# nju-ee/MODE-2022

Hardware: AMD Instinct MI355X
Metric: ERP stereo pairs/sec (512x1024, 192 disp) fwd+bwd (higher is better)
Workload: dtype fp32 storage/accumulate; products: 2xfp16 split (22-bit, per-tensor 2^k scale, 3 MFMAs) in the stride-1 3x3x3 / spherical / 3x3 layers incl. gradients (DESIGN 3u/3v); 3xbf16 split (24-bit, 6 MFMAs) in the stride-2 / transposed 3x3x3 layers and the polar spherical tiles (3j-3l); fp32 MFMA in the 32->; 1 GPU; ModeDisparity(192,Sphere,1024x512 Cassini) fwd+bwd+Adam step, batch 2/GPU (BASELINE configs[2]); global_batch=2, conv_arith=bf16x6, init=recipe state, seed 1 (tests/golden/recipe.py), parallelism=dp1

## Files before the change

mode-2022_amd/csrc/sphere_conv.hip:

```cpp
#include <cstring>

#include "common.h"
#include "sphere_internal.h"

namespace {

typedef float f32x16 __attribute__((ext_vector_type(16)));

constexpr int P = 64;
constexpr int CCH = 8;
constexpr int NTHREADS = 256;

struct Dims {
  int B, Ci, H, W, Co, KK, sH, sW, Ho, Wo, G;
  int Cig, Cog;
  int npix;
  int tps;
  int MT;
  int NCHUNK;
  int CB;
  int NB;
  int KSQ;
  int accumulate;
};
// ... 304 lines not shown
      for (int e = 0; e < s.y; ++e) {
        const int2 ent = entries[s.x + e];
        const float wt = __int_as_float(ent.y);
        v0 += wt * g0[ent.x];
        v1 += wt * g1[ent.x];
      }
      buf[((qd * 2) * d.KK + k) * P + p] = ok0 ? v0 : 0.f;
      buf[((qd * 2 + 1) * d.KK + k) * P + p] = ok1 ? v1 : 0.f;
    }
  };

  f32x16 acc0 = {0}, acc1 = {0};
  const float4* wpa = wp + ((long long)(g * MTc + (active ? mt : 0)) * NCHo) * d.KK * 64 + lane;

  produce(0, colbuf);
  __syncthreads();
  for (int ch = 0; ch < NCHo; ++ch) {
    float* cur = colbuf + (ch & 1) * rows * P;
    if (ch + 1 < NCHo) produce(ch + 1, colbuf + ((ch + 1) & 1) * rows * P);
    if (active) {
      const float4* wq = wpa + (long long)ch * d.KK * 64;
      const float* bp = cur + (lane >> 5) * P + (lane & 31);
      for (int quad = 0; quad < d.KK; ++quad) {
        const float4 a4 = wq[quad * 64];
        const float* bq = bp + quad * 8 * P;
        acc0 = mfma32(a4.x, bq[0], acc0);
        acc1 = mfma32(a4.x, bq[32], acc1);
        acc0 = mfma32(a4.y, bq[2 * P], acc0);
        acc1 = mfma32(a4.y, bq[2 * P + 32], acc1);
        acc0 = mfma32(a4.z, bq[4 * P], acc0);
        acc1 = mfma32(a4.z, bq[4 * P + 32], acc1);
        acc0 = mfma32(a4.w, bq[6 * P], acc0);
        acc1 = mfma32(a4.w, bq[6 * P + 32], acc1);
      }
    }
    __syncthreads();
  }

  if (active) {
    float* gxb = gx + ((long long)b * d.Ci + (long long)g * d.Cig) * HWin;
#pragma unroll
    for (int r = 0; r < 16; ++r) {
      const int c = mt * 32 + (r & 3) + 8 * (r >> 2) + 4 * (lane >> 5);
      if (c < d.Cig) {
        const int qq = q0 + (lane & 31);
        float* o0 = gxb + (long long)c * HWin + qq;
        if (qq < HWin) o0[0] = d.accumulate ? o0[0] + acc0[r] : acc0[r];
        if (qq + 32 < HWin) o0[32] = d.accumulate ? o0[32] + acc1[r] : acc1[r];
      }
    }
  }
}

__global__ __launch_bounds__(NTHREADS) void sphere_bwd_data_adj9_kernel(const float* __restrict__ gy, const int* __restrict__ rowptr,
                                                                         const int2* __restrict__ entries,
                                                                         const float4* __restrict__ wp, float* __restrict__ gx, Dims d,
                                                                         int MTc, int NCHo, int qtiles, const int* __restrict__ tile_list) {
  constexpr int KT = 9, EC = 4;
  extern __shared__ __attribute__((aligned(16))) char smem[];
  int4* ent_p = reinterpret_cast<int4*>(smem);
  float4* ent_w = reinterpret_cast<float4*>(smem + KT * P * 16);
  int2* span = reinterpret_cast<int2*>(smem + KT * P * 32);
  float* colbuf = reinterpret_cast<float*>(smem + KT * P * 40);
  constexpr int rows = CCH * KT;
  const int HWin = d.H * d.W;

  const int tile = xcd_remap(blockIdx.x, gridDim.x);
  const int b = tile / qtiles;
  const int q0 = (tile_list ? tile_list[tile - b * qtiles] : tile - b * qtiles) * P;
  const int g = blockIdx.z;
  const int tid = threadIdx.x;
  const int wave = tid >> 6, lane = tid & 63;
  const int mt = blockIdx.y * 4 + wave;
  const bool active = mt < MTc;

  for (int item = tid; item < KT * P; item += NTHREADS) {
    const int k = item / P, pp = item % P;
    const int qq = q0 + pp;
    int beg = 0, cnt = 0;
    if (qq < HWin) {
      beg = rowptr[(long long)k * HWin + qq];
      cnt = rowptr[(long long)k * HWin + qq + 1] - beg;
    }
    int pe[EC];
    float we[EC];
#pragma unroll
    for (int e = 0; e < EC; ++e) {
      const int2 ent = entries[beg + min(e, max(cnt - 1, 0))];
      pe[e] = e < cnt ? ent.x * 4 : 0;
      we[e] = e < cnt ? __int_as_float(ent.y) : 0.f;
    }
    ent_p[item] = make_int4(pe[0], pe[1], pe[2], pe[3]);
    ent_w[item] = make_float4(we[0], we[1], we[2], we[3]);
    span[item] = make_int2(beg, cnt);
  }
  __syncthreads();

  const int p = tid & (P - 1);
  static_assert(P == 64, "one wave per output-channel pair of the chunk");
  const int qd = __builtin_amdgcn_readfirstlane(tid / P);
  const float* gyg = gy + ((long long)b * d.Co + (long long)g * d.Cog) * d.npix;
  float lv[KT * 2 * EC];
  bool has_tail = false;
#pragma unroll
  for (int k = 0; k < KT; ++k) has_tail |= span[k * P + p].y > EC;

  auto issue = [&](int ch) {
    const int o0 = ch * CCH + qd * 2;
    const float* g0 = gyg + (long long)(o0 < d.Cog ? o0 : 0) * d.npix;
    const float* g1 = gyg + (long long)(o0 + 1 < d.Cog ? o0 + 1 : 0) * d.npix;
#pragma unroll
    for (int k = 0; k < KT; ++k) {
      const int4 pe = ent_p[k * P + p];
      const char* c0 = reinterpret_cast<const char*>(g0);
      const char* c1 = reinterpret_cast<const char*>(g1);
#define MODE_LD(base, off) (*reinterpret_cast<const float*>((base) + (unsigned)(off)))
      lv[k * 8 + 0] = MODE_LD(c0, pe.x); lv[k * 8 + 1] = MODE_LD(c0, pe.y); lv[k * 8 + 2] = MODE_LD(c0, pe.z); lv[k * 8 + 3] = MODE_LD(c0, pe.w);
      lv[k * 8 + 4] = MODE_LD(c1, pe.x); lv[k * 8 + 5] = MODE_LD(c1, pe.y); lv[k * 8 + 6] = MODE_LD(c1, pe.z); lv[k * 8 + 7] = MODE_LD(c1, pe.w);
#undef MODE_LD
    }
  };
  auto finish = [&](int ch, float* buf) {
    const int o0 = ch * CCH + qd * 2;
    const bool ok0 = o0 < d.Cog, ok1 = o0 + 1 < d.Cog;
    const float* g0 = gyg + (long long)(ok0 ? o0 : 0) * d.npix;
    const float* g1 = gyg + (long long)(ok1 ? o0 + 1 : 0) * d.npix;
    float v0[KT], v1[KT];
#pragma unroll
    for (int k = 0; k < KT; ++k) {
      const float4 we = ent_w[k * P + p];
      float a = we.x * lv[k * 8 + 0];
      float b = we.x * lv[k * 8 + 4];
      asm volatile("" : "+v"(a), "+v"(b));
      a = fmaf(we.y, lv[k * 8 + 1], a);
      b = fmaf(we.y, lv[k * 8 + 5], b);
      asm volatile("" : "+v"(a), "+v"(b));
      a = fmaf(we.z, lv[k * 8 + 2], a);
      b = fmaf(we.z, lv[k * 8 + 6], b);
      asm volatile("" : "+v"(a), "+v"(b));
      a = fmaf(we.w, lv[k * 8 + 3], a);
      b = fmaf(we.w, lv[k * 8 + 7], b);
      asm volatile("" : "+v"(a), "+v"(b));
      v0[k] = a;
      v1[k] = b;
    }
    if (has_tail) {
#pragma unroll
      for (int k = 0; k < KT; ++k) {
        const int2 s = span[k * P + p];
        for (int e = EC; e < s.y; ++e) {
          const int2 ent = entries[s.x + e];
          const float wt = __int_as_float(ent.y);
          float a = g0[ent.x], b = g1[ent.x];
          asm volatile("" : "+v"(a), "+v"(b));
          v0[k] = fmaf(wt, a, v0[k]);
          asm volatile("" : "+v"(v0[k]));
          v1[k] = fmaf(wt, b, v1[k]);
        }
      }
    }
#pragma unroll
    for (int k = 0; k < KT; ++k) {
      buf[((qd * 2) * KT + k) * P + p] = ok0 ? v0[k] : 0.f;
      buf[((qd * 2 + 1) * KT + k) * P + p] = ok1 ? v1[k] : 0.f;
    }
  };

  f32x16 acc0 = {0}, acc1 = {0};
  const float4* wpa = wp + ((long long)(g * MTc + (active ? mt : 0)) * NCHo) * KT * 64 + lane;

  float4 wcur[KT], wnxt[KT];
#pragma unroll
  for (int quad = 0; quad < KT; ++quad) wcur[quad] = wpa[quad * 64];
  issue(0);
  finish(0, colbuf);
  __syncthreads();
  for (int ch = 0; ch < NCHo; ++ch) {
    float* cur = colbuf + (ch & 1) * rows * P;
    float* nxt = colbuf + ((ch + 1) & 1) * rows * P;
    if (ch + 1 < NCHo) {
      const float4* wq = wpa + (long long)(ch + 1) * KT * 64;
#pragma unroll
      for (int quad = 0; quad < KT; ++quad) wnxt[quad] = wq[quad * 64];
      issue(ch + 1);
    }
    if (active) {
      const float* bp = cur + (lane >> 5) * P + (lane & 31);
      float bn[8];
#pragma unroll
      for (int i = 0; i < 8; ++i) bn[i] = bp[(i >> 1) * 2 * P + (i & 1) * 32];
#pragma unroll
      for (int quad = 0; quad < KT; ++quad) {
        const float4 a4 = wcur[quad];
        float bc[8];
#pragma unroll
        for (int i = 0; i < 8; ++i) bc[i] = bn[i];
        if (quad + 1 < KT) {
          const float* bq = bp + (quad + 1) * 8 * P;
#pragma unroll
          for (int i = 0; i < 8; ++i) bn[i] = bq[(i >> 1) * 2 * P + (i & 1) * 32];
        }
        __builtin_amdgcn_sched_barrier(0);
        acc0 = mfma32(a4.x, bc[0], acc0);
        acc1 = mfma32(a4.x, bc[1], acc1);
        acc0 = mfma32(a4.y, bc[2], acc0);
        acc1 = mfma32(a4.y, bc[3], acc1);
        acc0 = mfma32(a4.z, bc[4], acc0);
        acc1 = mfma32(a4.z, bc[5], acc1);
        acc0 = mfma32(a4.w, bc[6], acc0);
        acc1 = mfma32(a4.w, bc[7], acc1);
      }
    }
    if (ch + 1 < NCHo) {
      finish(ch + 1, nxt);
#pragma unroll
      for (int quad = 0; quad < KT; ++quad) wcur[quad] = wnxt[quad];
    }
    __syncthreads();
  }

  if (active) {
    float* gxb = gx + ((long long)b * d.Ci + (long long)g * d.Cig) * HWin;
#pragma unroll
    for (int r = 0; r < 16; ++r) {
      const int c = mt * 32 + (r & 3) + 8 * (r >> 2) + 4 * (lane >> 5);
      if (c < d.Cig) {
        const int qq = q0 + (lane & 31);
        float* o0 = gxb + (long long)c * HWin + qq;
        if (qq < HWin) o0[0] = d.accumulate ? o0[0] + acc0[r] : acc0[r];
        if (qq + 32 < HWin) o0[32] = d.accumulate ? o0[32] + acc1[r] : acc1[r];
      }
    }
  }
}

__global__ __launch_bounds__(NTHREADS) void sphere_bwd_data_kernel(const float* __restrict__ gy, const float* __restrict__ pos,
                                                                    const float4* __restrict__ wp, float* __restrict__ gx,
                                                                    Dims d) {
  extern __shared__ __attribute__((aligned(16))) char smem[];
  float4* tap_w = reinterpret_cast<float4*>(smem);
  unsigned* tap_off = reinterpret_cast<unsigned*>(smem + (size_t)d.KK * P * 16);
  float* gyl = reinterpret_cast<float*>(smem + (size_t)d.KK * P * 20);

  const int tile = xcd_remap(blockIdx.x, gridDim.x);
  const int b = tile / d.tps;
  const int pix0 = (tile - b * d.tps) * P;
  const int g = blockIdx.z;
  const int tid = threadIdx.x;
  const int wave = tid >> 6, lane = tid & 63;

  compute_tapinfo(pos, d, pix0, tap_off, tap_w);
  const float* gyb = gy + ((long long)b * d.Co + (long long)g * d.Cog) * d.npix;
  for (int idx = tid; idx < d.KSQ * 8 * P; idx += NTHREADS) {
    const int co = idx / P, p = idx % P;
    float v = 0.f;
    if (co < d.Cog && pix0 + p < d.npix) v = gyb[(long long)co * d.npix + pix0 + p];
    gyl[idx] = v;
  }
  __syncthreads();

  const long long HW = (long long)d.H * d.W;
  float* gxg = gx + ((long long)b * d.Ci + (long long)g * d.Cig) * HW;
  const float* bp = gyl + (lane >> 5) * P + (lane & 31);
  const int nrows = d.CB * d.KK;

  for (int nb = 0; nb < d.NB; ++nb) {
    f32x16 acc0 = {0}, acc1 = {0};
    const float4* wq = wp + ((long long)((g * d.NB + nb) * 4 + wave) * d.KSQ) * 64 + lane;
    for (int ks4 = 0; ks4 < d.KSQ; ++ks4) {
      const float4 a4 = wq[ks4 * 64];
      const float* bq = bp + ks4 * 8 * P;
      acc0 = mfma32(a4.x, bq[0], acc0);
      acc1 = mfma32(a4.x, bq[32], acc1);
      acc0 = mfma32(a4.y, bq[2 * P], acc0);
      acc1 = mfma32(a4.y, bq[2 * P + 32], acc1);
      acc0 = mfma32(a4.z, bq[4 * P], acc0);
      acc1 = mfma32(a4.z, bq[4 * P + 32], acc1);
      acc0 = mfma32(a4.w, bq[6 * P], acc0);
      acc1 = mfma32(a4.w, bq[6 * P + 32], acc1);
    }
#pragma unroll
    for (int r = 0; r < 16; ++r) {
      const int rr = wave * 32 + (r & 3) + 8 * (r >> 2) + 4 * (lane >> 5);
// ... 361 lines not shown
    for (int p = 0; p < npix; ++p) {
      const int n = corners(k, p, qs, ws);
      for (int i = 0; i < n; ++i) {
        const int32_t at = rowptr_host[(long long)k * HW + qs[i]]++;
        entries_host[2 * (long long)at] = p;
        int32_t bits;
        memcpy(&bits, &ws[i], 4);
        entries_host[2 * (long long)at + 1] = bits;
      }
    }
  for (long long i = nrows; i > 0; --i) rowptr_host[i] = rowptr_host[i - 1];
  rowptr_host[0] = 0;
  return MODE_OK;
}

static int bwd_data_adj_impl(const float* gy, const float* w, float* gx, float* wpack, const int32_t* adj_rowptr,
                             const int32_t* adj_entries, int B, int Ci, int H, int W, int Co, int Kh, int Kw, int Ho, int Wo, int groups,
                             int accumulate, const int32_t* tile_list, int n_list, mode_stream_t stream);

extern "C" int mode_sphere_conv_bwd_data_adj(const float* gy, const float* w, float* gx, float* wpack, const int32_t* adj_rowptr,
                                             const int32_t* adj_entries, int B, int Ci, int H, int W, int Co, int Kh, int Kw,
                                             int Ho, int Wo, int groups, int accumulate, mode_stream_t stream) {
  return bwd_data_adj_impl(gy, w, gx, wpack, adj_rowptr, adj_entries, B, Ci, H, W, Co, Kh, Kw, Ho, Wo, groups, accumulate, nullptr, 0, stream);
}

extern "C" int mode_sphere_conv_bwd_data_adj_list(const float* gy, const float* w, float* gx, float* wpack, const int32_t* adj_rowptr,
                                                  const int32_t* adj_entries, int B, int Ci, int H, int W, int Co, int Kh, int Kw,
                                                  int Ho, int Wo, int groups, int accumulate, const int32_t* tile_list, int n_list,
                                                  mode_stream_t stream) {
  MODE_REQUIRE(Kh * Kw == 9, MODE_ERR_UNSUPPORTED, "mode_sphere_conv_bwd_data_adj_list: 3x3 kernels only");
  MODE_REQUIRE(n_list >= 0 && (n_list == 0 || tile_list), MODE_ERR_BAD_ARG, "mode_sphere_conv_bwd_data_adj_list: bad tile list");
  if (n_list == 0) return MODE_OK;
  return bwd_data_adj_impl(gy, w, gx, wpack, adj_rowptr, adj_entries, B, Ci, H, W, Co, Kh, Kw, Ho, Wo, groups, accumulate, tile_list, n_list,
                           stream);
}

static int bwd_data_adj_impl(const float* gy, const float* w, float* gx, float* wpack, const int32_t* adj_rowptr,
                             const int32_t* adj_entries, int B, int Ci, int H, int W, int Co, int Kh, int Kw, int Ho, int Wo, int groups,
                             int accumulate, const int32_t* tile_list, int n_list, mode_stream_t stream) {
  Dims d;
  int rc = make_dims(d, B, Ci, H, W, Co, Kh, Kw, 1, 1, Ho, Wo, groups, "mode_sphere_conv_bwd_data_adj");
  if (rc != MODE_OK) return rc;
  d.accumulate = accumulate ? 1 : 0;
  if (B == 0) return MODE_OK;
  MODE_REQUIRE(gy && w && gx && wpack && adj_rowptr && adj_entries, MODE_ERR_BAD_ARG, "mode_sphere_conv_bwd_data_adj: null pointer");
  hipStream_t st = mode::as_stream(stream);
  const int MTc = mode::cdiv(d.Cig, 32);
  const int NCHo = mode::cdiv(d.Cog, CCH);
  const long long npack = (long long)d.G * MTc * NCHo * d.KK * 256;
  if (mode::pack_needed()) hipLaunchKernelGGL(pack_w_adj, dim3(mode::cdiv(npack, 256)), dim3(256), 0, st, w, wpack, d, MTc, NCHo);
  const int qtiles = tile_list ? n_list : mode::cdiv((long long)H * W, P);
  const dim3 grid(B * qtiles, mode::cdiv(MTc, 4), d.G);
  if (d.KK == 9) {
    const size_t lds = (size_t)9 * P * 40 + 2 * (size_t)CCH * 9 * P * 4;
    rc = mode::allow_lds(sphere_bwd_data_adj9_kernel, lds, "mode_sphere_conv_bwd_data_adj");
    if (rc != MODE_OK) return rc;
    hipLaunchKernelGGL(sphere_bwd_data_adj9_kernel, grid, dim3(NTHREADS), lds, st, gy, adj_rowptr,
                       reinterpret_cast<const int2*>(adj_entries), reinterpret_cast<const float4*>(wpack), gx, d, MTc, NCHo, qtiles, tile_list);
  } else {
    const size_t lds = (size_t)d.KK * P * 8 + 2 * (size_t)CCH * d.KK * P * 4;
    rc = mode::allow_lds(sphere_bwd_data_adj_kernel, lds, "mode_sphere_conv_bwd_data_adj");
    if (rc != MODE_OK) return rc;
    hipLaunchKernelGGL(sphere_bwd_data_adj_kernel, grid, dim3(NTHREADS), lds, st, gy, adj_rowptr,
                       reinterpret_cast<const int2*>(adj_entries), reinterpret_cast<const float4*>(wpack), gx, d, MTc, NCHo, qtiles);
  }
  return mode::check_launch("mode_sphere_conv_bwd_data_adj");
}
```

mode-2022_amd/csrc/sphere_conv_win.hip:

```cpp
#include <algorithm>
#include <cstring>
#include <vector>

#include "common.h"
#include "bn_internal.h"
#include "sphere_internal.h"
#include "sphere_tap.h"

namespace {

typedef float f32x16 __attribute__((ext_vector_type(16)));
typedef float f32x32 __attribute__((ext_vector_type(32)));

constexpr int RB = 2;
constexpr int TH = 32 * RB;
constexpr int TW = 4;
constexpr int WC = 8;
constexpr int CCH = 8;
constexpr int KT = 9;
constexpr int MTW = 4;
constexpr int NTHREADS = 64 * TW * RB;
constexpr int SROWS = NTHREADS / WC;
constexpr int WR_SMALL = TH + 17, WR_MID = TH + 81;
constexpr int WR_PIPE_MAX = 5 * SROWS;
// ... 1882 lines not shown
        const uint4* ga = reinterpret_cast<const uint4*>(gyb + (m8 * 32 + j) * BS_GP + 8 * ks8 + 4 * half);
        const uint4 a1 = ga[0], a2 = ga[128 * BS_GP / 4];
        if constexpr (F16) {
          acc8 = sp_mfma_f16(a2, b8[0], acc8);
          acc8 = sp_mfma_f16(a1, b8[1], acc8);
          acc8 = sp_mfma_f16(a1, b8[0], acc8);
        } else {
          const uint4 a3 = ga[2 * (128 * BS_GP / 4)];
          acc8 = sp_mfma(a3, b8[0], acc8);
          acc8 = sp_mfma(a1, b8[2], acc8);
          acc8 = sp_mfma(a2, b8[1], acc8);
          acc8 = sp_mfma(a2, b8[0], acc8);
          acc8 = sp_mfma(a1, b8[1], acc8);
          acc8 = sp_mfma(a1, b8[0], acc8);
        }
      }
      if (more_items) commit_xw(smem + (xbuf ^ 1) * BW_XW, wc);

      __syncthreads();
      if (have_next) commit_col(gpf[(wc + 1) & 1]);
      __syncthreads();
      if (have_next) sample(last_col ? smem + (xbuf ^ 1) * BW_XW : xw, prw0, pro0, b0);
    }
    cur = nxt;
    xbuf ^= 1;
  }
#undef MODE_BS_SPREAD

  float* pb = part + ((((long long)s * gridDim.z + blockIdx.z) * NCG + cg) * BW_SLOTS) * (128 * BW_CG);
#pragma unroll
  for (int m = 0; m < 4; ++m)
#pragma unroll
    for (int r = 0; r < 16; ++r) {
      const int o = m * 32 + (r & 3) + 8 * (r >> 2) + 4 * half;
      pb[((long long)wave * 128 + o) * BW_CG + j] = F16 ? acc[m][r] * unscale : acc[m][r];
    }
  float* red = smem;
  if (wave < 4) {
#pragma unroll
    for (int r = 0; r < 16; ++r) red[(m8 * 32 + (r & 3) + 8 * (r >> 2) + 4 * half) * BW_CG + j] = F16 ? acc8[r] * unscale : acc8[r];
  }
  __syncthreads();
  if (wave >= 4) {
#pragma unroll
    for (int r = 0; r < 16; ++r) red[(m8 * 32 + (r & 3) + 8 * (r >> 2) + 4 * half) * BW_CG + j] += F16 ? acc8[r] * unscale : acc8[r];
  }
  __syncthreads();
  for (int i = tid; i < 128 * BW_CG; i += NTHREADS) pb[(long long)8 * 128 * BW_CG + i] = red[i];
}

constexpr int BQ_X = ((BP_XW + 3) / 4) * 4;
constexpr int BQ_LDS_DWORDS = BQ_X + BS_GYB + 8 * BS_SCR;

__global__ __launch_bounds__(NTHREADS) void sphere_bww_polar_split_kernel(const float* __restrict__ gy, const float* __restrict__ x,
                                                                           float* __restrict__ part, WinDims d,
                                                                           const int* __restrict__ pitems, const float4* __restrict__ rec_w,
                                                                           const int* __restrict__ rec_off, int nitems, int S, int s_base) {
  extern __shared__ __attribute__((aligned(16))) float smem[];
  float* xw = smem;
  uint32_t* gyb = reinterpret_cast<uint32_t*>(smem + BQ_X);
  constexpr int WRP = BP_WR, CP = BP_CP;
  const int s = blockIdx.x, cg = blockIdx.y;
  const int g = blockIdx.z / d.MG, mg = blockIdx.z % d.MG;
  const int tid = threadIdx.x;
  const int wave = tid >> 6, lane = tid & 63;
  const int j = lane & 31, half = lane >> 5;
  float* scr = smem + BQ_X + BS_GYB + wave * BS_SCR;
  const long long HW = (long long)d.H * d.W;
  const int T = nitems * d.B;
  const int omax = d.Cog - mg * 128, cmax = d.Cig - cg * BW_CG;
  const int sh = half, sq = j >> 3, sp8 = j & 7;
  const int ks8 = wave >> 2, m8 = wave & 3;
  const int gpp = tid & 15, go0 = tid >> 4;

  f32x16 acc[4], acc8;
#pragma unroll
  for (int r = 0; r < 16; ++r) {
    acc[0][r] = acc[1][r] = acc[2][r] = acc[3][r] = 0.f;
    acc8[r] = 0.f;
  }
  for (int i = tid; i < BQ_LDS_DWORDS; i += NTHREADS) smem[i] = 0.f;

  constexpr int NE = KT * BP_TAPW;
  const int e0 = tid, e1 = tid + NTHREADS;
  const bool has1 = e1 < NE;
  const int k0 = e0 / BP_TAPW, k1 = (has1 ? e1 : 0) / BP_TAPW;
  const int col0 = (e0 % BP_TAPW) / BP_WR, r0 = e0 % BP_WR;
  const int col1 = ((has1 ? e1 : 0) % BP_TAPW) / BP_WR, r1 = (has1 ? e1 : 0) % BP_WR;

  auto sample = [&](const float4 w4, const int ro, uint4 (&bf)[3]) {
    const float* xb = xw + (8 * sq) * CP + ro;
    float v[8];
#pragma unroll
    for (int c = 0; c < 8; ++c) {
      const float* q = xb + c * CP;
      v[c] = __builtin_fmaf(w4.w, q[WRP + 1], __builtin_fmaf(w4.z, q[1], __builtin_fmaf(w4.y, q[WRP], w4.x * q[0])));
      asm("" : "+v"(v[c]));
    }
    float* sw = scr + (8 * sq) * BS_SCRP + 8 * sh + sp8;
#pragma unroll
    for (int c = 0; c < 8; ++c) sw[c * BS_SCRP] = v[c];
    const float* sr = scr + j * BS_SCRP + 8 * half;
    float t8[8];
#pragma unroll
    for (int i = 0; i < 8; ++i) t8[i] = sr[i];
    uint32_t q1[4], q2[4], q3[4];
#pragma unroll
    for (int i = 0; i < 4; ++i) sp_split2(t8[2 * i], t8[2 * i + 1], q1[i], q2[i], q3[i]);
    bf[0] = make_uint4(q1[0], q1[1], q1[2], q1[3]);
    bf[1] = make_uint4(q2[0], q2[1], q2[2], q2[3]);
    bf[2] = make_uint4(q3[0], q3[1], q3[2], q3[3]);
  };
  auto load_a = [&](int ks, uint4 (&a)[4][3]) {
#pragma unroll
    for (int m = 0; m < 4; ++m) {
      const uint4* ga = reinterpret_cast<const uint4*>(gyb + (m * 32 + j) * BS_GP + 8 * ks + 4 * half);
#pragma unroll
      for (int p = 0; p < 3; ++p) a[m][p] = ga[p * (128 * BS_GP / 4)];
    }
  };
  auto mma24 = [&](const uint4 (&a)[4][3], const uint4 (&bf)[3]) {
#define MODE_BS_TERM(PA, PB) _Pragma("unroll") for (int m = 0; m < 4; ++m) acc[m] = sp_mfma(a[m][PA], bf[PB], acc[m]);
    MODE_BS_TERM(2, 0)
    MODE_BS_TERM(0, 2)
    MODE_BS_TERM(1, 1)
    MODE_BS_TERM(1, 0)
    MODE_BS_TERM(0, 1)
    MODE_BS_TERM(0, 0)
#undef MODE_BS_TERM
  };

  for (int t = s; t < T; t += S) {
    const int b = t / nitems, it = t - b * nitems;
    const int* pi = pitems + (long long)it * BP_ITEM_INTS;
    const int h0 = pi[0], w = pi[1];
    __syncthreads();
    {
      const int rb0 = pi[2 + k0], cb0 = pi[2 + KT + k0], rb1 = pi[2 + k1], cb1 = pi[2 + KT + k1];
      const bool ok0 = cb0 + col0 < d.W, ok1 = has1 && cb1 + col1 < d.W;
      const float* xg = x + ((long long)b * d.Ci + (long long)g * d.Cig + (long long)cg * BW_CG) * HW;
      const long long a0 = ok0 ? (long long)((rb0 + r0) % d.H) * d.sh + (long long)(cb0 + col0) * d.sw : 0;
      const long long a1 = ok1 ? (long long)((rb1 + r1) % d.H) * d.sh + (long long)(cb1 + col1) * d.sw : 0;
#pragma unroll 1
      for (int c8 = 0; c8 < BW_CG; c8 += 8) {
        float v0[8], v1[8];
#pragma unroll
        for (int c = 0; c < 8; ++c) {
          const long long co = (long long)min(c8 + c, cmax - 1) * HW;
          v0[c] = xg[co + a0];
          v1[c] = xg[co + a1];
        }
#pragma unroll
        for (int c = 0; c < 8; ++c) {
          xw[(c8 + c) * BP_CP + e0] = (ok0 && c8 + c < cmax) ? v0[c] : 0.f;
          if (has1) xw[(c8 + c) * BP_CP + e1] = (ok1 && c8 + c < cmax) ? v1[c] : 0.f;
        }
      }
    }
    {
      const int h = h0 + 2 * gpp;
      const bool ok0 = h < d.H && w < d.W, ok1 = h + 1 < d.H && w < d.W;
      const float* gyb0 = gy + ((long long)b * d.Co + (long long)g * d.Cog + (long long)mg * 128) * HW +
                          (ok0 ? (long long)h * d.sh + (long long)w * d.sw : 0);
      const long long step1 = ok1 ? d.sh : 0;
      float v0[4], v1[4];
#pragma unroll
      for (int u = 0; u < 4; ++u) {
        const float* p = gyb0 + (long long)min(go0 + 32 * u, omax - 1) * HW;
        v0[u] = p[0];
        v1[u] = p[step1];
      }
#pragma unroll
      for (int u = 0; u < 4; ++u) {
        const bool oo = go0 + 32 * u < omax;
        uint32_t p1, p2, p3;
        sp_split2((ok0 && oo) ? v0[u] : 0.f, (ok1 && oo) ? v1[u] : 0.f, p1, p2, p3);
        uint32_t* dst = gyb + (go0 + 32 * u) * BS_GP + gpp;
        dst[0] = p1;
        dst[128 * BS_GP] = p2;
        dst[2 * 128 * BS_GP] = p3;
      }
    }
    const long long rbase = (long long)it * BW_NREC;
    const int px0 = 8 * sh + sp8;
    const float4 rw0 = rec_w[rbase + wave * BW_TH + px0], rw1 = rec_w[rbase + wave * BW_TH + 16 + px0];
    const float4 rw8 = rec_w[rbase + 8 * BW_TH + 16 * ks8 + px0];
    const int ro0 = rec_off[rbase + wave * BW_TH + px0], ro1 = rec_off[rbase + wave * BW_TH + 16 + px0];
    const int ro8 = rec_off[rbase + 8 * BW_TH + 16 * ks8 + px0];
    __syncthreads();
    uint4 a[4][3], b0[3], b1[3], b8[3];
    sample(rw0, ro0, b0);
    load_a(0, a);
    sample(rw1, ro1, b1);
    mma24(a, b0);
    load_a(1, a);
    sample(rw8, ro8, b8);
    mma24(a, b1);
    {
      const uint4* ga = reinterpret_cast<const uint4*>(gyb + (m8 * 32 + j) * BS_GP + 8 * ks8 + 4 * half);
      const uint4 a1 = ga[0], a2 = ga[128 * BS_GP / 4], a3 = ga[2 * (128 * BS_GP / 4)];
      acc8 = sp_mfma(a3, b8[0], acc8);
      acc8 = sp_mfma(a1, b8[2], acc8);
      acc8 = sp_mfma(a2, b8[1], acc8);
      acc8 = sp_mfma(a2, b8[0], acc8);
      acc8 = sp_mfma(a1, b8[1], acc8);
      acc8 = sp_mfma(a1, b8[0], acc8);
    }
  }
  __syncthreads();
  float* pb = part + ((((long long)(s_base + s) * gridDim.z + blockIdx.z) * gridDim.y + cg) * BW_SLOTS) * (128 * BW_CG);
#pragma unroll
  for (int m = 0; m < 4; ++m)
#pragma unroll
    for (int r = 0; r < 16; ++r) {
      const int o = m * 32 + (r & 3) + 8 * (r >> 2) + 4 * half;
      pb[((long long)wave * 128 + o) * BW_CG + j] = acc[m][r];
    }
  float* red = smem;
  if (wave < 4) {
#pragma unroll
    for (int r = 0; r < 16; ++r) red[(m8 * 32 + (r & 3) + 8 * (r >> 2) + 4 * half) * BW_CG + j] = acc8[r];
  }
  __syncthreads();
  if (wave >= 4) {
#pragma unroll
    for (int r = 0; r < 16; ++r) red[(m8 * 32 + (r & 3) + 8 * (r >> 2) + 4 * half) * BW_CG + j] += acc8[r];
  }
  __syncthreads();
  for (int i = tid; i < 128 * BW_CG; i += NTHREADS) pb[(long long)8 * 128 * BW_CG + i] = red[i];
}

size_t win_lds_bytes(int wr, bool pipe) { return ((size_t)(pipe ? 2 : 1) * CCH * chan_pitch(wr) + wr + 8) * sizeof(float); }
constexpr size_t TALL_W_BYTES = 2 * (size_t)MTW * 3 * 64 * sizeof(uint4);
size_t tall_split_lds_bytes(int wr) { return ((win_lds_bytes(wr, true) + 15) / 16) * 16 + TALL_W_BYTES; }
bool wrap_is_pipelined(int H) { return H + 1 <= WR_PIPE_MAX && win_lds_bytes(H + 1, true) <= 160 * 1024; }

__global__ __launch_bounds__(256) void transpose_planes_kernel(const float* __restrict__ in, float* __restrict__ out, int H, int W) {
  __shared__ float tile[32][33];
  const long long plane = (long long)blockIdx.z * H * W;
  const int w0 = blockIdx.x * 32, h0 = blockIdx.y * 32;
  const int tx = threadIdx.x & 31, ty = threadIdx.x >> 5;
#pragma unroll
  for (int i = 0; i < 32; i += 8) {
    const int h = h0 + ty + i, w = w0 + tx;
    if (h < H && w < W) tile[ty + i][tx] = in[plane + (long long)h * W + w];
  }
  __syncthreads();
#pragma unroll
  for (int i = 0; i < 32; i += 8) {
    const int w = w0 + ty + i, h = h0 + tx;
    if (h < H && w < W) out[plane + (long long)w * H + h] = tile[tx][ty + i];
  }
}

int make_win_dims(WinDims& d, int B, int Ci, int H, int W, int Co, int Kh, int Kw, int groups, const char* who) {
  MODE_REQUIRE(B >= 0 && Ci > 0 && H > 0 && W > 0 && Co > 0 && groups > 0, MODE_ERR_BAD_ARG, "%s: non-positive size", who);
  MODE_REQUIRE(Kh * Kw == KT, MODE_ERR_UNSUPPORTED, "%s: the windowed kernels are built for %d taps (got %dx%d)", who, KT, Kh, Kw);
  MODE_REQUIRE(Ci % groups == 0 && Co % groups == 0, MODE_ERR_BAD_ARG, "%s: channels not divisible by groups", who);
  MODE_REQUIRE((long long)H * W < (1LL << 30), MODE_ERR_UNSUPPORTED, "%s: image too large", who);
  d.B = B; d.Ci = Ci; d.H = H; d.W = W; d.Co = Co; d.G = groups;
  d.Cig = Ci / groups;
  d.Cog = Co / groups;
  d.NCH = mode::cdiv(d.Cig, CCH);
  d.MG = mode::cdiv(d.Cog, 128);
  d.wr = H + 1;
  d.sh = W;
  d.sw = 1;
  d.wrap_pipe = wrap_is_pipelined(H) ? 1 : 0;
  d.accumulate = 0;
  return MODE_OK;
}


}

extern "C" size_t mode_sphere_plan_max_tiles(int H, int W) {
  if (H <= 0 || W <= 0) return 0;
  return (size_t)mode::cdiv(H, TH) * mode::cdiv(W, TW);
}
// ... 414 lines not shown
  MODE_REQUIRE((amax_g == nullptr) == (amax_x == nullptr), MODE_ERR_BAD_ARG, "mode_sphere_conv_bwd_weight_win: both operand maxima, or neither");
  if (rc != MODE_OK) return rc;
  MODE_REQUIRE((gy_t == nullptr) == (x_t == nullptr), MODE_ERR_BAD_ARG, "mode_sphere_conv_bwd_weight_win: gy_t and x_t come together");
  if (gy_t) {
    d.sh = 1;
    d.sw = H;
  }
  MODE_REQUIRE(n_small >= 0 && n_mid >= 0 && n_wrap >= 0 && n_rest_pixels >= 0 && n_polar_items >= 0 &&
                   (size_t)n_small + n_mid + n_wrap == mode_sphere_plan_max_tiles(H, W),
               MODE_ERR_BAD_ARG, "mode_sphere_conv_bwd_weight_win: the plan must cover every tile");
  if (B == 0) return MODE_OK;
  MODE_REQUIRE(((gy && x) || (gy_t && n_rest_pixels == 0)) && pos && gw && workspace && tiles && (n_rest_pixels == 0 || rest_pixels) &&
                   (n_small == 0 || (rec_w && rec_off)) &&
                   (n_polar_items == 0 || (pitems && prec_w && prec_off)),
               MODE_ERR_BAD_ARG, "mode_sphere_conv_bwd_weight_win: null pointer");
  hipStream_t st = mode::as_stream(stream);
  const int NCG = mode::cdiv(d.Cig, BW_CG);
  const size_t slice = (size_t)d.G * d.MG * NCG * BW_SLOTS * 128 * BW_CG * sizeof(float);
  const float* gys = gy_t ? gy_t : gy;
  const float* xs = x_t ? x_t : x;
  int S = 0;
  if (n_small > 0) {
    S = bww_win_splits(d, n_small);
    if (split) {
      const size_t lds = (size_t)BS_LDS_DWORDS * sizeof(float);
      if (amax_g) {
        rc = mode::allow_lds(sphere_bww_split_kernel<true>, lds, "mode_sphere_conv_bwd_weight_win_split");
        if (rc != MODE_OK) return rc;
        hipLaunchKernelGGL(sphere_bww_split_kernel<true>, dim3(S, NCG, d.G * d.MG), dim3(NTHREADS), lds, st, gys, xs, workspace, d,
                           reinterpret_cast<const int4*>(tiles) + n_wrap + n_mid, reinterpret_cast<const float4*>(rec_w), rec_off, n_small, S,
                           amax_g, amax_x);
      } else {
        rc = mode::allow_lds(sphere_bww_split_kernel<false>, lds, "mode_sphere_conv_bwd_weight_win_split");
        if (rc != MODE_OK) return rc;
        hipLaunchKernelGGL(sphere_bww_split_kernel<false>, dim3(S, NCG, d.G * d.MG), dim3(NTHREADS), lds, st, gys, xs, workspace, d,
                           reinterpret_cast<const int4*>(tiles) + n_wrap + n_mid, reinterpret_cast<const float4*>(rec_w), rec_off, n_small, S,
                           amax_g, amax_x);
      }
    } else {
      const size_t lds = (size_t)BW_LDS_FLOATS * sizeof(float);
      rc = mode::allow_lds(sphere_bww_win_kernel, lds, "mode_sphere_conv_bwd_weight_win");
      if (rc != MODE_OK) return rc;
      hipLaunchKernelGGL(sphere_bww_win_kernel, dim3(S, NCG, d.G * d.MG), dim3(NTHREADS), lds, st, gys, xs, workspace, d,
                         reinterpret_cast<const int4*>(tiles) + n_wrap + n_mid, reinterpret_cast<const float4*>(rec_w), rec_off, n_small, S);
    }
    rc = mode::check_launch("mode_sphere_conv_bwd_weight_win");
    if (rc != MODE_OK) return rc;
  }
  int Sp = 0;
  if (n_polar_items > 0) {
    Sp = bww_polar_splits(d, n_polar_items);
    if (split) {
      const size_t lds = (size_t)BQ_LDS_DWORDS * sizeof(float);
      rc = mode::allow_lds(sphere_bww_polar_split_kernel, lds, "mode_sphere_conv_bwd_weight_win_split");
      if (rc != MODE_OK) return rc;
      hipLaunchKernelGGL(sphere_bww_polar_split_kernel, dim3(Sp, NCG, d.G * d.MG), dim3(NTHREADS), lds, st, gys, xs, workspace, d, pitems,
                         reinterpret_cast<const float4*>(prec_w), prec_off, n_polar_items, Sp, S);
    } else {
      const size_t lds = (size_t)BP_LDS_FLOATS * sizeof(float);
      rc = mode::allow_lds(sphere_bww_polar_kernel, lds, "mode_sphere_conv_bwd_weight_win");
      if (rc != MODE_OK) return rc;
      hipLaunchKernelGGL(sphere_bww_polar_kernel, dim3(Sp, NCG, d.G * d.MG), dim3(NTHREADS), lds, st, gys, xs, workspace, d, pitems,
                         reinterpret_cast<const float4*>(prec_w), prec_off, n_polar_items, Sp, S);
    }
    rc = mode::check_launch("mode_sphere_conv_bwd_weight_win(polar)");
    if (rc != MODE_OK) return rc;
  }
  if (S + Sp > 0) {
    const long long n = (long long)d.G * d.MG * NCG * KT * 128 * BW_CG;
    hipLaunchKernelGGL(reduce_gw_win, dim3(mode::cdiv(n, 256)), dim3(256), 0, st, workspace, gw, d, S + Sp, NCG);
    rc = mode::check_launch("mode_sphere_conv_bwd_weight_win(reduce)");
    if (rc != MODE_OK) return rc;
  }
  if (n_rest_pixels > 0)
    return mode::sphere_bwd_weight_general(gy, pos, x, gw, reinterpret_cast<float*>(reinterpret_cast<char*>(workspace) + slice * (S + Sp)), B,
                                           Ci, H, W, Co, Kh, Kw, 1, 1, H, W, groups, rest_pixels, n_rest_pixels, st,
                                           "mode_sphere_conv_bwd_weight_win(rest)");
  return MODE_OK;
}

extern "C" int mode_transpose_planes(const float* in, float* out, long long planes, int H, int W, mode_stream_t stream) {
  MODE_REQUIRE(planes >= 0 && H > 0 && W > 0, MODE_ERR_BAD_ARG, "mode_transpose_planes: bad size");
  if (planes == 0) return MODE_OK;
  MODE_REQUIRE(in && out, MODE_ERR_BAD_ARG, "mode_transpose_planes: null pointer");
  hipStream_t st = mode::as_stream(stream);
  for (long long p0 = 0; p0 < planes; p0 += 65535) {
    const int np = (int)std::min<long long>(65535, planes - p0);
    hipLaunchKernelGGL(transpose_planes_kernel, dim3(mode::cdiv(W, 32), mode::cdiv(H, 32), np), dim3(256), 0, st,
                       in + p0 * (long long)H * W, out + p0 * (long long)H * W, H, W);
  }
  return mode::check_launch("mode_transpose_planes");
}

namespace {

constexpr int AJ_PIX = TH * TW;

template <int NS, bool F16>
__device__ __forceinline__ void bwd_data_tile(const float* __restrict__ gy, const uint4* __restrict__ wps, float* __restrict__ gx,
                                              const WinDims& d , int NCH16, const int4 t,
                                              const int4* __restrict__ rec_off, const float4* __restrict__ rec_w,
                                              const int2* __restrict__ rec_off2, const float2* __restrict__ rec_w2, float* smem,
                                              float sx, float unscale) {
  constexpr int WRP = WR_SMALL, CP = SP_CP;
  uint4* opbuf = reinterpret_cast<uint4*>(smem + SP_WIN_FLOATS);
  const int h0 = t.x, w0 = t.y, rbase = t.z, cbase = t.w & 0xffff;
  const int b = blockIdx.y;
  const int g = blockIdx.z / d.MG, mg = blockIdx.z % d.MG;
  const int tid = threadIdx.x, wave = tid >> 6, lane = tid & 63, half = lane >> 5;
  const long long HW = (long long)d.H * d.W;
// ... 634 lines not shown
```

Measured before the change: 35.67 pairs/s.

## Halve adj9 backward-data tile to 32 pixels; add opt-in fp16 polar weight-grad kernel

The 9-tap adjacency backward-data kernel now handles 32-pixel half tiles, giving each thread one output channel instead of two and launching twice as many blocks. This shrinks per-thread register and LDS footprint and should raise occupancy, at the cost of duplicated weight loads and per-block setup. Separately, the polar split weight-gradient kernel is templated with an fp16 2-term split path (3 MFMAs instead of 6) that uses per-tensor scales. That path is enabled only through the MODE_SPHERE_POLAR_F16 environment variable.

```diff
diff --git a/mode-2022_amd/csrc/sphere_conv.hip b/mode-2022_amd/csrc/sphere_conv.hip
--- a/mode-2022_amd/csrc/sphere_conv.hip
+++ b/mode-2022_amd/csrc/sphere_conv.hip
@@ -380,30 +380,35 @@
   }
 }
 
+constexpr int PH = 32;
 __global__ __launch_bounds__(NTHREADS) void sphere_bwd_data_adj9_kernel(const float* __restrict__ gy, const int* __restrict__ rowptr,
                                                                          const int2* __restrict__ entries,
                                                                          const float4* __restrict__ wp, float* __restrict__ gx, Dims d,
                                                                          int MTc, int NCHo, int qtiles, const int* __restrict__ tile_list) {
   constexpr int KT = 9, EC = 4;
+  static_assert(NTHREADS == CCH * PH, "one thread per (output channel of the chunk, pixel of the half tile)");
+  static_assert(P == 2 * PH, "two half tiles per listed tile");
   extern __shared__ __attribute__((aligned(16))) char smem[];
   int4* ent_p = reinterpret_cast<int4*>(smem);
-  float4* ent_w = reinterpret_cast<float4*>(smem + KT * P * 16);
-  int2* span = reinterpret_cast<int2*>(smem + KT * P * 32);
-  float* colbuf = reinterpret_cast<float*>(smem + KT * P * 40);
+  float4* ent_w = reinterpret_cast<float4*>(smem + KT * PH * 16);
+  int2* span = reinterpret_cast<int2*>(smem + KT * PH * 32);
+  float* colbuf = reinterpret_cast<float*>(smem + KT * PH * 40);
   constexpr int rows = CCH * KT;
   const int HWin = d.H * d.W;
 
-  const int tile = xcd_remap(blockIdx.x, gridDim.x);
-  const int b = tile / qtiles;
-  const int q0 = (tile_list ? tile_list[tile - b * qtiles] : tile - b * qtiles) * P;
+  const int htile = xcd_remap(blockIdx.x, gridDim.x);
+  const int b = htile / (2 * qtiles);
+  const int hrem = htile - b * 2 * qtiles;
+  const int q0 = (tile_list ? tile_list[hrem >> 1] : hrem >> 1) * P + (hrem & 1) * PH;
+  if (q0 >= HWin) return;
   const int g = blockIdx.z;
   const int tid = threadIdx.x;
   const int wave = tid >> 6, lane = tid & 63;
   const int mt = blockIdx.y * 4 + wave;
   const bool active = mt < MTc;
 
-  for (int item = tid; item < KT * P; item += NTHREADS) {
-    const int k = item / P, pp = item % P;
+  for (int item = tid; item < KT * PH; item += NTHREADS) {
+    const int k = item / PH, pp = item % PH;
     const int qq = q0 + pp;
     int beg = 0, cnt = 0;
     if (qq < HWin) {
@@ -424,77 +429,62 @@
   }
   __syncthreads();
 
-  const int p = tid & (P - 1);
-  static_assert(P == 64, "one wave per output-channel pair of the chunk");
-  const int qd = __builtin_amdgcn_readfirstlane(tid / P);
+  const int p = tid & (PH - 1);
+  const int cc = tid / PH;
   const float* gyg = gy + ((long long)b * d.Co + (long long)g * d.Cog) * d.npix;
-  float lv[KT * 2 * EC];
+  float lv[KT * EC];
   bool has_tail = false;
 #pragma unroll
-  for (int k = 0; k < KT; ++k) has_tail |= span[k * P + p].y > EC;
+  for (int k = 0; k < KT; ++k) has_tail |= span[k * PH + p].y > EC;
 
   auto issue = [&](int ch) {
-    const int o0 = ch * CCH + qd * 2;
-    const float* g0 = gyg + (long long)(o0 < d.Cog ? o0 : 0) * d.npix;
-    const float* g1 = gyg + (long long)(o0 + 1 < d.Cog ? o0 + 1 : 0) * d.npix;
+    const int o0 = ch * CCH + cc;
+    const char* c0 = reinterpret_cast<const char*>(gyg + (long long)(o0 < d.Cog ? o0 : 0) * d.npix);
 #pragma unroll
     for (int k = 0; k < KT; ++k) {
-      const int4 pe = ent_p[k * P + p];
-      const char* c0 = reinterpret_cast<const char*>(g0);
-      const char* c1 = reinterpret_cast<const char*>(g1);
+      const int4 pe = ent_p[k * PH + p];
 #define MODE_LD(base, off) (*reinterpret_cast<const float*>((base) + (unsigned)(off)))
-      lv[k * 8 + 0] = MODE_LD(c0, pe.x); lv[k * 8 + 1] = MODE_LD(c0, pe.y); lv[k * 8 + 2] = MODE_LD(c0, pe.z); lv[k * 8 + 3] = MODE_LD(c0, pe.w);
-      lv[k * 8 + 4] = MODE_LD(c1, pe.x); lv[k * 8 + 5] = MODE_LD(c1, pe.y); lv[k * 8 + 6] = MODE_LD(c1, pe.z); lv[k * 8 + 7] = MODE_LD(c1, pe.w);
+      lv[k * 4 + 0] = MODE_LD(c0, pe.x); lv[k * 4 + 1] = MODE_LD(c0, pe.y); lv[k * 4 + 2] = MODE_LD(c0, pe.z); lv[k * 4 + 3] = MODE_LD(c0, pe.w);
 #undef MODE_LD
     }
   };
   auto finish = [&](int ch, float* buf) {
-    const int o0 = ch * CCH + qd * 2;
-    const bool ok0 = o0 < d.Cog, ok1 = o0 + 1 < d.Cog;
+    const int o0 = ch * CCH + cc;
+    const bool ok0 = o0 < d.Cog;
     const float* g0 = gyg + (long long)(ok0 ? o0 : 0) * d.npix;
-    const float* g1 = gyg + (long long)(ok1 ? o0 + 1 : 0) * d.npix;
-    float v0[KT], v1[KT];
+    float v0[KT];
 #pragma unroll
     for (int k = 0; k < KT; ++k) {
-      const float4 we = ent_w[k * P + p];
-      float a = we.x * lv[k * 8 + 0];
-      float b = we.x * lv[k * 8 + 4];
-      asm volatile("" : "+v"(a), "+v"(b));
-      a = fmaf(we.y, lv[k * 8 + 1], a);
-      b = fmaf(we.y, lv[k * 8 + 5], b);
-      asm volatile("" : "+v"(a), "+v"(b));
-      a = fmaf(we.z, lv[k * 8 + 2], a);
-      b = fmaf(we.z, lv[k * 8 + 6], b);
-      asm volatile("" : "+v"(a), "+v"(b));
-      a = fmaf(we.w, lv[k * 8 + 3], a);
-      b = fmaf(we.w, lv[k * 8 + 7], b);
-      asm volatile("" : "+v"(a), "+v"(b));
+      const float4 we = ent_w[k * PH + p];
+      float a = we.x * lv[k * 4 + 0];
+      asm volatile("" : "+v"(a));
+      a = fmaf(we.y, lv[k * 4 + 1], a);
+      asm volatile("" : "+v"(a));
+      a = fmaf(we.z, lv[k * 4 + 2], a);
+      asm volatile("" : "+v"(a));
+      a = fmaf(we.w, lv[k * 4 + 3], a);
+      asm volatile("" : "+v"(a));
       v0[k] = a;
-      v1[k] = b;
     }
     if (has_tail) {
 #pragma unroll
       for (int k = 0; k < KT; ++k) {
-        const int2 s = span[k * P + p];
+        const int2 s = span[k * PH + p];
         for (int e = EC; e < s.y; ++e) {
           const int2 ent = entries[s.x + e];
           const float wt = __int_as_float(ent.y);
-          float a = g0[ent.x], b = g1[ent.x];
-          asm volatile("" : "+v"(a), "+v"(b));
+          float a = g0[ent.x];
+          asm volatile("" : "+v"(a));
           v0[k] = fmaf(wt, a, v0[k]);
           asm volatile("" : "+v"(v0[k]));
-          v1[k] = fmaf(wt, b, v1[k]);
         }
       }
     }
 #pragma unroll
-    for (int k = 0; k < KT; ++k) {
-      buf[((qd * 2) * KT + k) * P + p] = ok0 ? v0[k] : 0.f;
-      buf[((qd * 2 + 1) * KT + k) * P + p] = ok1 ? v1[k] : 0.f;
-    }
+    for (int k = 0; k < KT; ++k) buf[(cc * KT + k) * PH + p] = ok0 ? v0[k] : 0.f;
   };
 
-  f32x16 acc0 = {0}, acc1 = {0};
+  f32x16 acc0 = {0};
   const float4* wpa = wp + ((long long)(g * MTc + (active ? mt : 0)) * NCHo) * KT * 64 + lane;
 
   float4 wcur[KT], wnxt[KT];
@@ -504,8 +494,8 @@
   finish(0, colbuf);
   __syncthreads();
   for (int ch = 0; ch < NCHo; ++ch) {
-    float* cur = colbuf + (ch & 1) * rows * P;
-    float* nxt = colbuf + ((ch + 1) & 1) * rows * P;
+    float* cur = colbuf + (ch & 1) * rows * PH;
+    float* nxt = colbuf + ((ch + 1) & 1) * rows * PH;
     if (ch + 1 < NCHo) {
       const float4* wq = wpa + (long long)(ch + 1) * KT * 64;
 #pragma unroll
@@ -513,30 +503,26 @@
       issue(ch + 1);
     }
     if (active) {
-      const float* bp = cur + (lane >> 5) * P + (lane & 31);
-      float bn[8];
-#pragma unroll
-      for (int i = 0; i < 8; ++i) bn[i] = bp[(i >> 1) * 2 * P + (i & 1) * 32];
+      const float* bp = cur + (lane >> 5) * PH + (lane & 31);
+      float bn[4];
+#pragma unroll
+      for (int i = 0; i < 4; ++i) bn[i] = bp[i * 2 * PH];
 #pragma unroll
       for (int quad = 0; quad < KT; ++quad) {
         const float4 a4 = wcur[quad];
-        float bc[8];
-#pragma unroll
-        for (int i = 0; i < 8; ++i) bc[i] = bn[i];
+        float bc[4];
+#pragma unroll
+        for (int i = 0; i < 4; ++i) bc[i] = bn[i];
         if (quad + 1 < KT) {
-          const float* bq = bp + (quad + 1) * 8 * P;
-#pragma unroll
-          for (int i = 0; i < 8; ++i) bn[i] = bq[(i >> 1) * 2 * P + (i & 1) * 32];
+          const float* bq = bp + (quad + 1) * 8 * PH;
+#pragma unroll
+          for (int i = 0; i < 4; ++i) bn[i] = bq[i * 2 * PH];
         }
         __builtin_amdgcn_sched_barrier(0);
         acc0 = mfma32(a4.x, bc[0], acc0);
-        acc1 = mfma32(a4.x, bc[1], acc1);
-        acc0 = mfma32(a4.y, bc[2], acc0);
-        acc1 = mfma32(a4.y, bc[3], acc1);
-        acc0 = mfma32(a4.z, bc[4], acc0);
-        acc1 = mfma32(a4.z, bc[5], acc1);
-        acc0 = mfma32(a4.w, bc[6], acc0);
-        acc1 = mfma32(a4.w, bc[7], acc1);
+        acc0 = mfma32(a4.y, bc[1], acc0);
+        acc0 = mfma32(a4.z, bc[2], acc0);
+        acc0 = mfma32(a4.w, bc[3], acc0);
       }
     }
     if (ch + 1 < NCHo) {
@@ -549,14 +535,13 @@
 
   if (active) {
     float* gxb = gx + ((long long)b * d.Ci + (long long)g * d.Cig) * HWin;
+    const int qq = q0 + (lane & 31);
 #pragma unroll
     for (int r = 0; r < 16; ++r) {
       const int c = mt * 32 + (r & 3) + 8 * (r >> 2) + 4 * (lane >> 5);
-      if (c < d.Cig) {
-        const int qq = q0 + (lane & 31);
+      if (c < d.Cig && qq < HWin) {
         float* o0 = gxb + (long long)c * HWin + qq;
-        if (qq < HWin) o0[0] = d.accumulate ? o0[0] + acc0[r] : acc0[r];
-        if (qq + 32 < HWin) o0[32] = d.accumulate ? o0[32] + acc1[r] : acc1[r];
+        o0[0] = d.accumulate ? o0[0] + acc0[r] : acc0[r];
       }
     }
   }
@@ -1024,10 +1009,12 @@
   const int qtiles = tile_list ? n_list : mode::cdiv((long long)H * W, P);
   const dim3 grid(B * qtiles, mode::cdiv(MTc, 4), d.G);
   if (d.KK == 9) {
-    const size_t lds = (size_t)9 * P * 40 + 2 * (size_t)CCH * 9 * P * 4;
+    MODE_REQUIRE((long long)B * qtiles * 2 < (1ll << 31), MODE_ERR_UNSUPPORTED, "mode_sphere_conv_bwd_data_adj: too many tiles");
+    const dim3 grid9(B * qtiles * 2, mode::cdiv(MTc, 4), d.G);
+    const size_t lds = (size_t)9 * PH * 40 + 2 * (size_t)CCH * 9 * PH * 4;
     rc = mode::allow_lds(sphere_bwd_data_adj9_kernel, lds, "mode_sphere_conv_bwd_data_adj");
     if (rc != MODE_OK) return rc;
-    hipLaunchKernelGGL(sphere_bwd_data_adj9_kernel, grid, dim3(NTHREADS), lds, st, gy, adj_rowptr,
+    hipLaunchKernelGGL(sphere_bwd_data_adj9_kernel, grid9, dim3(NTHREADS), lds, st, gy, adj_rowptr,
                        reinterpret_cast<const int2*>(adj_entries), reinterpret_cast<const float4*>(wpack), gx, d, MTc, NCHo, qtiles, tile_list);
   } else {
     const size_t lds = (size_t)d.KK * P * 8 + 2 * (size_t)CCH * d.KK * P * 4;
diff --git a/mode-2022_amd/csrc/sphere_conv_win.hip b/mode-2022_amd/csrc/sphere_conv_win.hip
--- a/mode-2022_amd/csrc/sphere_conv_win.hip
+++ b/mode-2022_amd/csrc/sphere_conv_win.hip
@@ -1958,11 +1958,21 @@
 constexpr int BQ_X = ((BP_XW + 3) / 4) * 4;
 constexpr int BQ_LDS_DWORDS = BQ_X + BS_GYB + 8 * BS_SCR;
 
+template <bool F16>
 __global__ __launch_bounds__(NTHREADS) void sphere_bww_polar_split_kernel(const float* __restrict__ gy, const float* __restrict__ x,
                                                                            float* __restrict__ part, WinDims d,
                                                                            const int* __restrict__ pitems, const float4* __restrict__ rec_w,
-                                                                           const int* __restrict__ rec_off, int nitems, int S, int s_base) {
+                                                                           const int* __restrict__ rec_off, int nitems, int S, int s_base,
+                                                                           const float* __restrict__ amax_g,
+                                                                           const float* __restrict__ amax_x) {
   extern __shared__ __attribute__((aligned(16))) float smem[];
+  float sg = 1.f, sx = 1.f, unscale = 1.f;
+  if (F16) {
+    sg = sp_f16_scale_of(mode::absmax_load(amax_g));
+    sx = sp_f16_scale_of(mode::absmax_load(amax_x));
+    unscale = (1.f / sg) * (1.f / sx);
+  }
+  constexpr int NPC = F16 ? 2 : 3;
   float* xw = smem;
   uint32_t* gyb = reinterpret_cast<uint32_t*>(smem + BQ_X);
   constexpr int WRP = BP_WR, CP = BP_CP;
@@ -1994,9 +2004,10 @@
   const int col0 = (e0 % BP_TAPW) / BP_WR, r0 = e0 % BP_WR;
   const int col1 = ((has1 ? e1 : 0) % BP_TAPW) / BP_WR, r1 = (has1 ? e1 : 0) % BP_WR;
 
-  auto sample = [&](const float4 w4, const int ro, uint4 (&bf)[3]) {
+  auto sample = [&](const float4 w4_, const int ro, uint4 (&bf)[3]) {
     const float* xb = xw + (8 * sq) * CP + ro;
     float v[8];
+    const float4 w4 = F16 ? make_float4(w4_.x * sx, w4_.y * sx, w4_.z * sx, w4_.w * sx) : w4_;
 #pragma unroll
     for (int c = 0; c < 8; ++c) {
       const float* q = xb + c * CP;
@@ -2011,29 +2022,42 @@
 #pragma unroll
     for (int i = 0; i < 8; ++i) t8[i] = sr[i];
     uint32_t q1[4], q2[4], q3[4];
-#pragma unroll
-    for (int i = 0; i < 4; ++i) sp_split2(t8[2 * i], t8[2 * i + 1], q1[i], q2[i], q3[i]);
+    if constexpr (F16) {
+#pragma unroll
+      for (int i = 0; i < 4; ++i) sp_split2_f16(t8[2 * i], t8[2 * i + 1], q1[i], q2[i]);
+    } else {
+#pragma unroll
+      for (int i = 0; i < 4; ++i) sp_split2(t8[2 * i], t8[2 * i + 1], q1[i], q2[i], q3[i]);
+      bf[2] = make_uint4(q3[0], q3[1], q3[2], q3[3]);
+    }
     bf[0] = make_uint4(q1[0], q1[1], q1[2], q1[3]);
     bf[1] = make_uint4(q2[0], q2[1], q2[2], q2[3]);
-    bf[2] = make_uint4(q3[0], q3[1], q3[2], q3[3]);
   };
   auto load_a = [&](int ks, uint4 (&a)[4][3]) {
 #pragma unroll
     for (int m = 0; m < 4; ++m) {
       const uint4* ga = reinterpret_cast<const uint4*>(gyb + (m * 32 + j) * BS_GP + 8 * ks + 4 * half);
 #pragma unroll
-      for (int p = 0; p < 3; ++p) a[m][p] = ga[p * (128 * BS_GP / 4)];
+      for (int p = 0; p < NPC; ++p) a[m][p] = ga[p * (128 * BS_GP / 4)];
     }
   };
   auto mma24 = [&](const uint4 (&a)[4][3], const uint4 (&bf)[3]) {
+    if constexpr (F16) {
+#define MODE_BS_TERM(PA, PB) _Pragma("unroll") for (int m = 0; m < 4; ++m) acc[m] = sp_mfma_f16(a[m][PA], bf[PB], acc[m]);
+      MODE_BS_TERM(1, 0)
+      MODE_BS_TERM(0, 1)
+      MODE_BS_TERM(0, 0)
+#undef MODE_BS_TERM
+    } else {
 #define MODE_BS_TERM(PA, PB) _Pragma("unroll") for (int m = 0; m < 4; ++m) acc[m] = sp_mfma(a[m][PA], bf[PB], acc[m]);
-    MODE_BS_TERM(2, 0)
-    MODE_BS_TERM(0, 2)
-    MODE_BS_TERM(1, 1)
-    MODE_BS_TERM(1, 0)
-    MODE_BS_TERM(0, 1)
-    MODE_BS_TERM(0, 0)
+      MODE_BS_TERM(2, 0)
+      MODE_BS_TERM(0, 2)
+      MODE_BS_TERM(1, 1)
+      MODE_BS_TERM(1, 0)
+      MODE_BS_TERM(0, 1)
+      MODE_BS_TERM(0, 0)
 #undef MODE_BS_TERM
+    }
   };
 
   for (int t = s; t < T; t += S) {
@@ -2080,11 +2104,16 @@
       for (int u = 0; u < 4; ++u) {
         const bool oo = go0 + 32 * u < omax;
         uint32_t p1, p2, p3;
-        sp_split2((ok0 && oo) ? v0[u] : 0.f, (ok1 && oo) ? v1[u] : 0.f, p1, p2, p3);
+        const float ga = (ok0 && oo) ? v0[u] : 0.f, gb = (ok1 && oo) ? v1[u] : 0.f;
         uint32_t* dst = gyb + (go0 + 32 * u) * BS_GP + gpp;
+        if constexpr (F16) {
+          sp_split2_f16(ga * sg, gb * sg, p1, p2);
+        } else {
+          sp_split2(ga, gb, p1, p2, p3);
+          dst[2 * 128 * BS_GP] = p3;
+        }
         dst[0] = p1;
         dst[128 * BS_GP] = p2;
-        dst[2 * 128 * BS_GP] = p3;
       }
     }
     const long long rbase = (long long)it * BW_NREC;
@@ -2104,13 +2133,20 @@
     mma24(a, b1);
     {
       const uint4* ga = reinterpret_cast<const uint4*>(gyb + (m8 * 32 + j) * BS_GP + 8 * ks8 + 4 * half);
-      const uint4 a1 = ga[0], a2 = ga[128 * BS_GP / 4], a3 = ga[2 * (128 * BS_GP / 4)];
-      acc8 = sp_mfma(a3, b8[0], acc8);
-      acc8 = sp_mfma(a1, b8[2], acc8);
-      acc8 = sp_mfma(a2, b8[1], acc8);
-      acc8 = sp_mfma(a2, b8[0], acc8);
-      acc8 = sp_mfma(a1, b8[1], acc8);
-      acc8 = sp_mfma(a1, b8[0], acc8);
+      const uint4 a1 = ga[0], a2 = ga[128 * BS_GP / 4];
+      if constexpr (F16) {
+        acc8 = sp_mfma_f16(a2, b8[0], acc8);
+        acc8 = sp_mfma_f16(a1, b8[1], acc8);
+        acc8 = sp_mfma_f16(a1, b8[0], acc8);
+      } else {
+        const uint4 a3 = ga[2 * (128 * BS_GP / 4)];
+        acc8 = sp_mfma(a3, b8[0], acc8);
+        acc8 = sp_mfma(a1, b8[2], acc8);
+        acc8 = sp_mfma(a2, b8[1], acc8);
+        acc8 = sp_mfma(a2, b8[0], acc8);
+        acc8 = sp_mfma(a1, b8[1], acc8);
+        acc8 = sp_mfma(a1, b8[0], acc8);
+      }
     }
   }
   __syncthreads();
@@ -2120,17 +2156,17 @@
 #pragma unroll
     for (int r = 0; r < 16; ++r) {
       const int o = m * 32 + (r & 3) + 8 * (r >> 2) + 4 * half;
-      pb[((long long)wave * 128 + o) * BW_CG + j] = acc[m][r];
+      pb[((long long)wave * 128 + o) * BW_CG + j] = F16 ? acc[m][r] * unscale : acc[m][r];
     }
   float* red = smem;
   if (wave < 4) {
 #pragma unroll
-    for (int r = 0; r < 16; ++r) red[(m8 * 32 + (r & 3) + 8 * (r >> 2) + 4 * half) * BW_CG + j] = acc8[r];
+    for (int r = 0; r < 16; ++r) red[(m8 * 32 + (r & 3) + 8 * (r >> 2) + 4 * half) * BW_CG + j] = F16 ? acc8[r] * unscale : acc8[r];
   }
   __syncthreads();
   if (wave >= 4) {
 #pragma unroll
-    for (int r = 0; r < 16; ++r) red[(m8 * 32 + (r & 3) + 8 * (r >> 2) + 4 * half) * BW_CG + j] += acc8[r];
+    for (int r = 0; r < 16; ++r) red[(m8 * 32 + (r & 3) + 8 * (r >> 2) + 4 * half) * BW_CG + j] += F16 ? acc8[r] * unscale : acc8[r];
   }
   __syncthreads();
   for (int i = tid; i < 128 * BW_CG; i += NTHREADS) pb[(long long)8 * 128 * BW_CG + i] = red[i];
@@ -2651,10 +2687,18 @@
     Sp = bww_polar_splits(d, n_polar_items);
     if (split) {
       const size_t lds = (size_t)BQ_LDS_DWORDS * sizeof(float);
-      rc = mode::allow_lds(sphere_bww_polar_split_kernel, lds, "mode_sphere_conv_bwd_weight_win_split");
-      if (rc != MODE_OK) return rc;
-      hipLaunchKernelGGL(sphere_bww_polar_split_kernel, dim3(Sp, NCG, d.G * d.MG), dim3(NTHREADS), lds, st, gys, xs, workspace, d, pitems,
-                         reinterpret_cast<const float4*>(prec_w), prec_off, n_polar_items, Sp, S);
+      static const char* polar_env = getenv("MODE_SPHERE_POLAR_F16");
+      if (amax_g && polar_env && polar_env[0] == '1') {
+        rc = mode::allow_lds(sphere_bww_polar_split_kernel<true>, lds, "mode_sphere_conv_bwd_weight_win_split");
+        if (rc != MODE_OK) return rc;
+        hipLaunchKernelGGL(sphere_bww_polar_split_kernel<true>, dim3(Sp, NCG, d.G * d.MG), dim3(NTHREADS), lds, st, gys, xs, workspace, d,
+                           pitems, reinterpret_cast<const float4*>(prec_w), prec_off, n_polar_items, Sp, S, amax_g, amax_x);
+      } else {
+        rc = mode::allow_lds(sphere_bww_polar_split_kernel<false>, lds, "mode_sphere_conv_bwd_weight_win_split");
+        if (rc != MODE_OK) return rc;
+        hipLaunchKernelGGL(sphere_bww_polar_split_kernel<false>, dim3(Sp, NCG, d.G * d.MG), dim3(NTHREADS), lds, st, gys, xs, workspace, d,
+                           pitems, reinterpret_cast<const float4*>(prec_w), prec_off, n_polar_items, Sp, S, nullptr, nullptr);
+      }
     } else {
       const size_t lds = (size_t)BP_LDS_FLOATS * sizeof(float);
       rc = mode::allow_lds(sphere_bww_polar_kernel, lds, "mode_sphere_conv_bwd_weight_win");
```

New measurement: 35.72 pairs/s, median of 6. Within noise of the previous version (+0.1%).
